# databendlabs/databend

Measured on AMD Instinct MI355X. Metric: rows/s TPC-H Q1 hash-agg, higher is better.
Workload: dtype i64/i128 decimal

## Files before the change

databend_amd/csrc/k_decimal.hip:

```cpp
#include "dev_common.h"
#include "dev_decimal.h"
#include "dev_load.h"
#include "runtime.h"

using namespace dbhip;

namespace {

struct DecParams : DecOp {
  const void* a;
  const void* b;
  void* out;
  const uint8_t* a_validity;
  const uint8_t* b_validity;
  int64_t a_voff, b_voff;
  int64_t n;
  uint32_t* err_words;
  unsigned long long* err_count;
  int a_type, b_type, out_type;
  int a_scalar, b_scalar;
};

__device__ __forceinline__ i128 load_operand(const void* p, int type, bool scalar, int64_t i) {
  int64_t j = scalar ? 0 : i;
  switch (type) {
    case DBHIP_T_DEC128: return ((const i128*)p)[j];
    case DBHIP_T_DEC256: return ((const i128*)p)[2 * j];
    case DBHIP_T_DEC64: case DBHIP_T_I64: return (i128)((const int64_t*)p)[j];
    case DBHIP_T_I8: return (i128)((const int8_t*)p)[j];
    case DBHIP_T_I16: return (i128)((const int16_t*)p)[j];
    case DBHIP_T_I32: return (i128)((const int32_t*)p)[j];
    case DBHIP_T_U8: return (i128)((const uint8_t*)p)[j];
    case DBHIP_T_U16: return (i128)((const uint16_t*)p)[j];
    case DBHIP_T_U32: return (i128)((const uint32_t*)p)[j];
    default: return (i128)((const uint64_t*)p)[j];
  }
}

__device__ __forceinline__ void dec_raise(const DecParams& p, int64_t row) {
  if (p.a_validity && !bit_get(p.a_validity, p.a_voff + (p.a_scalar ? 0 : row))) return;
  if (p.b_validity && !bit_get(p.b_validity, p.b_voff + (p.b_scalar ? 0 : row))) return;
  if (p.err_words) atomicAnd(&p.err_words[row >> 5], ~(1u << (row & 31)));
  if (p.err_count) atomicAdd(p.err_count, 1ULL);
}

template <int N>
__device__ __forceinline__ void load_operand_n(const void* p, int type, bool scalar, const int64_t (&i)[N], i128 (&out)[N]) {
  int64_t j[N];
#pragma unroll
  for (int u = 0; u < N; ++u) j[u] = scalar ? 0 : i[u];
  switch (type) {
    case DBHIP_T_DEC128:
#pragma unroll
      for (int u = 0; u < N; ++u) out[u] = ((const i128*)p)[j[u]];
      break;
    case DBHIP_T_DEC256:
#pragma unroll
      for (int u = 0; u < N; ++u) out[u] = ((const i128*)p)[2 * j[u]];
      break;
    case DBHIP_T_DEC64: case DBHIP_T_I64:
#pragma unroll
      for (int u = 0; u < N; ++u) out[u] = (i128)((const int64_t*)p)[j[u]];
      break;
    case DBHIP_T_I8:
#pragma unroll
      for (int u = 0; u < N; ++u) out[u] = (i128)((const int8_t*)p)[j[u]];
      break;
    case DBHIP_T_I16:
#pragma unroll
      for (int u = 0; u < N; ++u) out[u] = (i128)((const int16_t*)p)[j[u]];
      break;
    case DBHIP_T_I32:
#pragma unroll
      for (int u = 0; u < N; ++u) out[u] = (i128)((const int32_t*)p)[j[u]];
      break;
    case DBHIP_T_U8:
#pragma unroll
      for (int u = 0; u < N; ++u) out[u] = (i128)((const uint8_t*)p)[j[u]];
      break;
    case DBHIP_T_U16:
#pragma unroll
      for (int u = 0; u < N; ++u) out[u] = (i128)((const uint16_t*)p)[j[u]];
      break;
    case DBHIP_T_U32:
#pragma unroll
      for (int u = 0; u < N; ++u) out[u] = (i128)((const uint32_t*)p)[j[u]];
      break;
    default:
#pragma unroll
      for (int u = 0; u < N; ++u) out[u] = (i128)((const uint64_t*)p)[j[u]];
      break;
  }
}

__global__ __launch_bounds__(256) void decimal_kernel(DecParams p) {
  const bool t128 = p.t_is_128;
  const bool a_dec = p.a_type == DBHIP_T_DEC64 || p.a_type == DBHIP_T_DEC128 || p.a_type == DBHIP_T_DEC256;
  const bool b_dec = p.b_type == DBHIP_T_DEC64 || p.b_type == DBHIP_T_DEC128 || p.b_type == DBHIP_T_DEC256;
  constexpr int U = 4;
  const int64_t T = (int64_t)gridDim.x * blockDim.x;
  const int64_t t = (int64_t)blockIdx.x * blockDim.x + threadIdx.x;
  for (int64_t base = 0; base < p.n; base += U * T) {
    int64_t row[U];
    bool in[U];
#pragma unroll
    for (int u = 0; u < U; ++u) {
      row[u] = base + u * T + t;
      in[u] = row[u] < p.n;
      if (!in[u]) row[u] = p.n - 1;
    }
    i128 av[U], bv[U];
    load_operand_n<U>(p.a, p.a_type, p.a_scalar, row, av);
    load_operand_n<U>(p.b, p.b_type, p.b_scalar, row, bv);
#pragma unroll
    for (int u = 0; u < U; ++u) {
      if (!in[u]) continue;
      const int64_t i = row[u];
      i128 r;
      if (!dec_row(p, av[u], bv[u], a_dec, b_dec, t128, &r)) {
        dec_raise(p, i);
        r = 1;
      }
      if (p.out_type == DBHIP_T_DEC128) ((i128*)p.out)[i] = r;
      else ((int64_t*)p.out)[i] = (int64_t)r;
    }
  }
}

struct DSize {
  int p, s;
};

bool decimal_props(int type, int prec, int scale, DSize* out) {
  switch (type) {
    case DBHIP_T_DEC64: case DBHIP_T_DEC128: case DBHIP_T_DEC256: *out = {prec, scale}; return prec >= 1 && prec <= 76 && scale <= prec;
    case DBHIP_T_I8: case DBHIP_T_U8: *out = {3, 0}; return true;
    case DBHIP_T_I16: case DBHIP_T_U16: *out = {5, 0}; return true;
    case DBHIP_T_I32: case DBHIP_T_U32: *out = {10, 0}; return true;
    case DBHIP_T_I64: *out = {19, 0}; return true;
    case DBHIP_T_U64: *out = {20, 0}; return true;
  }
  return false;
}

inline int imin(int a, int b) { return a < b ? a : b; }
inline int imax(int a, int b) { return a > b ? a : b; }

bool result_size(int op, DSize a, DSize b, DSize* left, DSize* right, DSize* ret) {
  int precision, scale;
  int la = a.p - a.s, lb = b.p - b.s;
  switch (op) {
    case DBHIP_OP_MULTIPLY:
      scale = imin(a.s + b.s, imax(imax(a.s, b.s), 12));
      precision = la + lb + scale;
      break;
    case DBHIP_OP_DIVIDE:
      scale = imax(a.s, imin(a.s + 6, 12));
      precision = la + b.s + scale;
      break;
    case DBHIP_OP_PLUS:
    case DBHIP_OP_MINUS:
      scale = imax(a.s, b.s);
      precision = imax(la, lb) + scale + 1;
      break;
    default:
      return false;
  }
  precision = imin(precision, (a.p <= 38 && b.p <= 38) ? 38 : 76);
  if (precision < 1 || scale > precision) return false;
  *ret = {precision, scale};
  switch (op) {
    case DBHIP_OP_MULTIPLY:
      *left = {precision, a.s};
      *right = {precision, b.s};
      break;
    case DBHIP_OP_DIVIDE: {
      int pp = imax(precision, imax(a.p, b.p));
      *left = {pp, a.s};
      *right = {pp, b.s};
    } break;
    default:
      *left = *ret;
      *right = *ret;
  }
  return left->s <= left->p && right->s <= right->p;
}

}

namespace dbhip {
int32_t decimal256_arith(int32_t op, const dbhip_col* lhs, const dbhip_col* rhs, int64_t n, int32_t out_type, uint8_t out_precision,
                         uint8_t out_scale, void* out, uint8_t* err_bitmap, uint64_t* err_count_dev, void* stream);
}

extern "C" {

int32_t dbhip_decimal_result_size(int32_t op, uint8_t lp, uint8_t ls, uint8_t rp, uint8_t rs,
                                  uint8_t* out_precision_host, uint8_t* out_scale_host) {
  DSize l, r, ret;
  if (!result_size(op, {lp, ls}, {rp, rs}, &l, &r, &ret)) {
    set_error("dbhip_decimal_result_size: no decimal result for op %d on (%d,%d),(%d,%d)", op, lp, ls, rp, rs);
    return DBHIP_ERR_INVALID;
  }
  if (out_precision_host) *out_precision_host = (uint8_t)ret.p;
  if (out_scale_host) *out_scale_host = (uint8_t)ret.s;
  return DBHIP_OK;
}

int32_t dbhip_decimal_arith(int32_t op, const dbhip_col* lhs, const dbhip_col* rhs, int64_t n,
                            int32_t out_type, uint8_t out_precision, uint8_t out_scale, void* out,
                            uint8_t* err_bitmap, uint64_t* err_count_dev, void* stream) {
  DBHIP_REQUIRE(lhs && rhs && (out || n == 0), "dbhip_decimal_arith: NULL argument");
  if (out_precision > 38)
    return decimal256_arith(op, lhs, rhs, n, out_type, out_precision, out_scale, out, err_bitmap, err_count_dev, stream);
  DecParams p;
  int want_type, rp, rs;
  int32_t rc = dbhip_decimal_decode_internal(op, lhs->type, lhs->precision, lhs->scale, rhs->type, rhs->precision, rhs->scale, &p,
                                             &want_type, &rp, &rs);
  if (rc) return rc;
  if (rp != out_precision || rs != out_scale || want_type != out_type) {
    set_error("dbhip_decimal_arith: result is type %d Decimal(%d,%d); caller passed type %d Decimal(%d,%d)",
              want_type, rp, rs, out_type, out_precision, out_scale);
    return DBHIP_ERR_INVALID;
  }
  hipStream_t s = resolve_stream(stream);
  if (err_bitmap) DBHIP_CHECK(hipMemsetAsync(err_bitmap, 0xFF, (size_t)ceil_div(n, 32) * 4, s));
  if (n == 0) return DBHIP_OK;
  p.a = lhs->data; p.b = rhs->data; p.out = out;
  p.a_validity = lhs->validity; p.b_validity = rhs->validity;
  p.a_voff = lhs->validity_offset; p.b_voff = rhs->validity_offset;
  p.n = n;
  p.err_words = (uint32_t*)err_bitmap;
  p.err_count = (unsigned long long*)err_count_dev;
  p.a_type = lhs->type; p.b_type = rhs->type; p.out_type = out_type;
  p.a_scalar = lhs->is_scalar; p.b_scalar = rhs->is_scalar;
  hipLaunchKernelGGL(decimal_kernel, dim3(grid_for(ceil_div(n, 4), 256, 1024)), dim3(256), 0, s, p);
  DBHIP_LAUNCH_CHECK();
  return DBHIP_OK;
}

}

int32_t dbhip_decimal_decode_internal(int op, int a_type, int a_prec, int a_scale, int b_type, int b_prec, int b_scale,
                                      DecOp* out, int* out_type, int* out_precision, int* out_scale) {
  DSize a, b, left, right, ret;
  if (!decimal_props(a_type, a_prec, a_scale, &a) || !decimal_props(b_type, b_prec, b_scale, &b)) {
    set_error("decimal arithmetic: operand types (%d,%d) have no decimal properties", a_type, b_type);
    return DBHIP_ERR_INVALID;
  }
  const bool a_dec = a_type == DBHIP_T_DEC64 || a_type == DBHIP_T_DEC128 || a_type == DBHIP_T_DEC256;
  const bool b_dec = b_type == DBHIP_T_DEC64 || b_type == DBHIP_T_DEC128 || b_type == DBHIP_T_DEC256;
  DBHIP_REQUIRE(a_dec || b_dec, "decimal arithmetic: at least one side must be decimal");
  if (!result_size(op, a, b, &left, &right, &ret)) {
    set_error("decimal arithmetic: unsupported op %d", op);
    return DBHIP_ERR_INVALID;
  }
  if (ret.p > 38) {
    set_error("decimal arithmetic: Decimal(%d,%d) results (T = i256) are evaluated by dbhip_decimal_arith, not inside fused programs", ret.p, ret.s);
    return DBHIP_ERR_UNSUPPORTED;
  }
  DecOp& p = *out;
  p.op = op;
  p.a_from_scale = a.s; p.a_to_scale = left.s; p.a_to_precision = left.p;
  p.a_check = a_dec ? (a.s != left.s) : 1;
  p.b_from_scale = b.s; p.b_to_scale = right.s; p.b_to_precision = right.p;
  p.b_check = b_dec ? (b.s != right.s) : 1;
  p.t_is_128 = ret.p > 18;
  p.ret_precision = ret.p; p.ret_scale = ret.s;
  p.overflow = ret.p == (p.t_is_128 ? 38 : 18);
  p.scale_mul = op == DBHIP_OP_MULTIPLY ? a.s + b.s - ret.s
                                        : (op == DBHIP_OP_DIVIDE ? b.s + ret.s - a.s : 0);
  if (p.scale_mul < 0 || p.scale_mul > 38) {
    set_error("decimal arithmetic: scale shift %d outside the supported range", p.scale_mul);
    return DBHIP_ERR_UNSUPPORTED;
  }
  {
    const bool pass_a = a_dec ? !p.a_check : p.a_to_scale == 0, pass_b = b_dec ? !p.b_check : p.b_to_scale == 0;
    p.trivial = pass_a && pass_b && (((op == DBHIP_OP_PLUS || op == DBHIP_OP_MINUS) && !p.overflow) || (op == DBHIP_OP_MULTIPLY && p.scale_mul == 0));
  }
  *out_type = ret.p <= 18 ? DBHIP_T_DEC64 : DBHIP_T_DEC128;
  *out_precision = ret.p;
  *out_scale = ret.s;
  return DBHIP_OK;
}
```

Before: 90.72 billion.

## Add specialized fast decimal add/sub/mul kernel with templated operand kinds

Adds a templated fast-path decimal kernel for plus, minus and multiply without division. It specializes on operand kind (scalar, 64-bit, 128-bit, narrow int) and result width, precomputes rescale factors on the host, and uses vectorized 16-byte loads and stores in a grid-stride chunked loop. The aim is to remove the runtime type dispatch and generic 128-bit arithmetic of the general kernel. In exchange it adds many template instantiations, alignment requirements, and a duplicated overflow and rescale logic path that must match the generic semantics.

After: 90.71 billion (median of 2 runs). Within noise of the previous version (-0.0%).

```diff
diff --git a/databend_amd/csrc/dev_decimal_fast.h b/databend_amd/csrc/dev_decimal_fast.h
--- /dev/null
+++ b/databend_amd/csrc/dev_decimal_fast.h
@@ -0,0 +1,123 @@
+#pragma once
+#include "dev_decimal.h"
+
+struct DecFastSide {
+  i128 mul;
+  i128 max;
+  int rescale;
+  int uns;
+};
+
+struct DecFastOp {
+  DecFastSide a, b;
+  i128 ret_max;
+  int overflow;
+};
+
+__host__ inline bool dec_fast_decode(const DecOp& p, bool a_dec, bool b_dec, bool a_u64, bool b_u64, DecFastOp* f) {
+  if (dec_op_needs_division(p)) return false;
+  const bool ra = a_dec ? p.a_check != 0 : p.a_to_scale != 0, rb = b_dec ? p.b_check != 0 : p.b_to_scale != 0;
+  if (p.op == DBHIP_OP_MULTIPLY && (ra || rb)) return false;
+  const int ka = a_dec ? p.a_to_scale - p.a_from_scale : p.a_to_scale, kb = b_dec ? p.b_to_scale - p.b_from_scale : p.b_to_scale;
+  if ((ra && (ka < 0 || ka > 38)) || (rb && (kb < 0 || kb > 38))) return false;
+  if (!p.t_is_128 && ((ra && ka > 18) || (rb && kb > 18))) return false;
+  f->a = {ra ? pow10_i128(ka) : (i128)1, max_for_precision(p.a_to_precision), ra, a_u64};
+  f->b = {rb ? pow10_i128(kb) : (i128)1, max_for_precision(p.b_to_precision), rb, b_u64};
+  f->ret_max = max_for_precision(p.ret_precision);
+  f->overflow = p.overflow;
+  return true;
+}
+
+__host__ __device__ __forceinline__ bool decf_convert(const DecFastSide& s, int64_t x, int64_t* out) {
+  if (!s.rescale) {
+    *out = x;
+    return true;
+  }
+  const i128 r = (i128)x * (i128)(int64_t)s.mul;
+  *out = (int64_t)r;
+  return r <= s.max && r >= -s.max;
+}
+
+__host__ __device__ __forceinline__ bool decf_mag_mul64(uint64_t ax, u128 f, u128 max, u128* out) {
+  const u128 lo = (u128)ax * (uint64_t)f;
+  const u128 hi = (u128)ax * (uint64_t)(f >> 64) + (uint64_t)(lo >> 64);
+  *out = (hi << 64) | (uint64_t)lo;
+  return (uint64_t)(hi >> 64) == 0 && *out <= max;
+}
+__host__ __device__ __forceinline__ bool decf_mag_mul128(u128 ax, u128 f, u128 max, u128* out) {
+  const u256 pr = u256_mul_128(ax, f);
+  *out = pr.lo;
+  return pr.hi == 0 && pr.lo <= max;
+}
+
+__host__ __device__ __forceinline__ bool decf_convert(const DecFastSide& s, int64_t x, i128* out) {
+  const bool neg = !s.uns && x < 0;
+  if (!s.rescale) {
+    *out = (i128)(((u128)(neg ? ~0ULL : 0ULL) << 64) | (uint64_t)x);
+    return true;
+  }
+  u128 m;
+  const bool ok = decf_mag_mul64(neg ? (uint64_t)0 - (uint64_t)x : (uint64_t)x, (u128)s.mul, (u128)s.max, &m);
+  *out = neg ? (i128)((u128)0 - m) : (i128)m;
+  return ok;
+}
+__host__ __device__ __forceinline__ bool decf_convert(const DecFastSide& s, i128 x, i128* out) {
+  if (!s.rescale) {
+    *out = x;
+    return true;
+  }
+  const bool neg = x < 0;
+  u128 m;
+  const bool ok = decf_mag_mul128(neg ? (u128)0 - (u128)x : (u128)x, (u128)s.mul, (u128)s.max, &m);
+  *out = neg ? (i128)((u128)0 - m) : (i128)m;
+  return ok;
+}
+
+__host__ __device__ __forceinline__ i128 decf_mul128(int64_t a, bool a_uns, int64_t b, bool b_uns) {
+  const u128 p = (u128)(uint64_t)a * (uint64_t)b;
+  uint64_t hi = (uint64_t)(p >> 64);
+  if (!a_uns && a < 0) hi -= (uint64_t)b;
+  if (!b_uns && b < 0) hi -= (uint64_t)a;
+  return (i128)(((u128)hi << 64) | (uint64_t)p);
+}
+__host__ __device__ __forceinline__ i128 decf_mul128(i128 a, bool, int64_t b, bool b_uns) {
+  const uint64_t al = (uint64_t)(u128)a, ah = (uint64_t)((u128)a >> 64);
+  const u128 p = (u128)al * (uint64_t)b;
+  uint64_t hi = (uint64_t)(p >> 64) + ah * (uint64_t)b;
+  if (!b_uns && b < 0) hi -= al;
+  return (i128)(((u128)hi << 64) | (uint64_t)p);
+}
+__host__ __device__ __forceinline__ i128 decf_mul128(int64_t a, bool a_uns, i128 b, bool b_uns) { return decf_mul128(b, b_uns, a, a_uns); }
+__host__ __device__ __forceinline__ i128 decf_mul128(i128 a, bool, i128 b, bool) { return (i128)((u128)a * (u128)b); }
+
+template <typename T>
+struct decf_unsigned;
+template <>
+struct decf_unsigned<int64_t> {
+  typedef uint64_t type;
+};
+template <>
+struct decf_unsigned<i128> {
+  typedef u128 type;
+};
+
+template <typename T, int OP, bool A_PRE, bool B_PRE, typename AT, typename BT>
+__host__ __device__ __forceinline__ bool dec_row_fast(const DecFastOp& p, AT av, bool a_ok, BT bv, bool b_ok, T* out) {
+  typedef typename decf_unsigned<T>::type UT;
+  if constexpr (OP == DBHIP_OP_MULTIPLY) {
+    if constexpr (sizeof(T) == 8) *out = (T)((UT)av * (UT)bv);
+    else *out = decf_mul128(av, p.a.uns != 0, bv, p.b.uns != 0);
+    return (A_PRE ? a_ok : true) & (B_PRE ? b_ok : true);
+  } else {
+    T a, b;
+    bool ok = true;
+    if constexpr (A_PRE) { a = (T)av; ok = a_ok; }
+    else ok = decf_convert(p.a, av, &a);
+    if constexpr (B_PRE) { b = (T)bv; ok = b_ok & ok; }
+    else ok = decf_convert(p.b, bv, &b) & ok;
+    const T t = OP == DBHIP_OP_PLUS ? (T)((UT)a + (UT)b) : (T)((UT)a - (UT)b);
+    if (p.overflow) ok = ok & (t <= (T)p.ret_max) & (t >= -(T)p.ret_max);
+    *out = t;
+    return ok;
+  }
+}
diff --git a/databend_amd/csrc/k_decimal.hip b/databend_amd/csrc/k_decimal.hip
--- a/databend_amd/csrc/k_decimal.hip
+++ b/databend_amd/csrc/k_decimal.hip
@@ -1,5 +1,6 @@
 #include "dev_common.h"
 #include "dev_decimal.h"
+#include "dev_decimal_fast.h"
 #include "dev_load.h"
 #include "runtime.h"
 
@@ -125,6 +126,193 @@
       else ((int64_t*)p.out)[i] = (int64_t)r;
     }
   }
+}
+
+enum { DK_SCALAR = 0, DK_C64 = 1, DK_C128 = 2, DK_NARROW = 3 };
+constexpr int DF_BLOCK = 256;
+constexpr int DF_PAIRS = 4;
+constexpr int DF_CHUNK_ROWS = DF_BLOCK * 2 * DF_PAIRS;
+constexpr int DF_GRID_CAP = 512;
+
+struct DecFastParams : DecParams {
+  DecFastOp f;
+};
+
+typedef int64_t df_i64x2 __attribute__((ext_vector_type(2)));
+typedef uint32_t df_u32x4 __attribute__((ext_vector_type(4)));
+
+template <int K, typename T> struct df_operand { typedef int64_t type; };
+template <typename T> struct df_operand<DK_C128, T> { typedef i128 type; };
+template <typename T> struct df_operand<DK_SCALAR, T> { typedef T type; };
+
+__device__ __forceinline__ int64_t df_load_narrow(const void* p, int type, int64_t i) {
+  switch (type) {
+    case DBHIP_T_I8: return ((const int8_t*)p)[i];
+    case DBHIP_T_I16: return ((const int16_t*)p)[i];
+    case DBHIP_T_I32: return ((const int32_t*)p)[i];
+    case DBHIP_T_U8: return ((const uint8_t*)p)[i];
+    case DBHIP_T_U16: return ((const uint16_t*)p)[i];
+    default: return ((const uint32_t*)p)[i];
+  }
+}
+
+__device__ __forceinline__ i128 df_i128(df_u32x4 w) {
+  return (i128)(((u128)(((uint64_t)w.w << 32) | w.z) << 64) | (((uint64_t)w.y << 32) | w.x));
+}
+__device__ __forceinline__ df_u32x4 df_words(i128 v) {
+  const uint64_t lo = (uint64_t)(u128)v, hi = (uint64_t)((u128)v >> 64);
+  df_u32x4 w = {(uint32_t)lo, (uint32_t)(lo >> 32), (uint32_t)hi, (uint32_t)(hi >> 32)};
+  return w;
+}
+
+template <int K, typename V>
+__device__ __forceinline__ void df_load_chunk(const void* base, int type, int64_t chunk, uint32_t tid, V (&v)[2 * DF_PAIRS]) {
+  if constexpr (K == DK_C64) {
+    const char* cb = (const char*)base + chunk * (int64_t)(DF_CHUNK_ROWS * 8);
+#pragma unroll
+    for (int u = 0; u < DF_PAIRS; ++u) {
+      const df_i64x2 x = *(const df_i64x2*)(cb + (uint32_t)((u * DF_BLOCK + tid) * 16u));
+      v[2 * u] = x.x;
+      v[2 * u + 1] = x.y;
+    }
+  } else if constexpr (K == DK_C128) {
+    const char* cb = (const char*)base + chunk * (int64_t)(DF_CHUNK_ROWS * 16);
+#pragma unroll
+    for (int k = 0; k < 2 * DF_PAIRS; ++k)
+            v[k] = df_i128(*(const df_u32x4*)(cb + (uint32_t)((((k >> 1) * DF_BLOCK + tid) * 2u + (k & 1)) * 16u)));
+  } else if constexpr (K == DK_NARROW) {
+    const int64_t r0 = chunk * DF_CHUNK_ROWS;
+#pragma unroll
+    for (int k = 0; k < 2 * DF_PAIRS; ++k) v[k] = df_load_narrow(base, type, r0 + ((k >> 1) * DF_BLOCK + tid) * 2 + (k & 1));
+  }
+}
+
+template <int K, typename V>
+__device__ __forceinline__ V df_load_row(const void* base, int type, int64_t row) {
+  if constexpr (K == DK_C64) return ((const int64_t*)base)[row];
+  else if constexpr (K == DK_C128) return ((const i128*)base)[row];
+  else return df_load_narrow(base, type, row);
+}
+
+template <typename T, int OP, int AK, int BK>
+__global__ __launch_bounds__(DF_BLOCK) void decimal_fast_kernel(DecFastParams p) {
+  typedef typename df_operand<AK, T>::type AT;
+  typedef typename df_operand<BK, T>::type BT;
+  constexpr bool A_PRE = AK == DK_SCALAR, B_PRE = BK == DK_SCALAR;
+  const uint32_t tid = threadIdx.x;
+  T sa = 0, sb = 0;
+  bool a_ok = true, b_ok = true;
+  if constexpr (A_PRE) {
+    const bool a_dec = p.a_type == DBHIP_T_DEC64 || p.a_type == DBHIP_T_DEC128;
+    i128 c = 0;
+    a_ok = convert_operand(load_operand(p.a, p.a_type, true, 0), a_dec, p.a_from_scale, p.a_to_scale, p.a_to_precision, p.a_check, sizeof(T) == 16, &c);
+    sa = (T)c;
+  }
+  if constexpr (B_PRE) {
+    const bool b_dec = p.b_type == DBHIP_T_DEC64 || p.b_type == DBHIP_T_DEC128;
+    i128 c = 0;
+    b_ok = convert_operand(load_operand(p.b, p.b_type, true, 0), b_dec, p.b_from_scale, p.b_to_scale, p.b_to_precision, p.b_check, sizeof(T) == 16, &c);
+    sb = (T)c;
+  }
+  const int64_t n_chunks = (p.n + DF_CHUNK_ROWS - 1) / DF_CHUNK_ROWS;
+  for (int64_t chunk = blockIdx.x; chunk < n_chunks; chunk += gridDim.x) {
+    const int64_t r0 = chunk * DF_CHUNK_ROWS;
+    if (r0 + DF_CHUNK_ROWS <= p.n) {
+      AT av[2 * DF_PAIRS];
+      BT bv[2 * DF_PAIRS];
+      if constexpr (A_PRE) {
+#pragma unroll
+        for (int k = 0; k < 2 * DF_PAIRS; ++k) av[k] = sa;
+      } else {
+        df_load_chunk<AK>(p.a, p.a_type, chunk, tid, av);
+      }
+      if constexpr (B_PRE) {
+#pragma unroll
+        for (int k = 0; k < 2 * DF_PAIRS; ++k) bv[k] = sb;
+      } else {
+        df_load_chunk<BK>(p.b, p.b_type, chunk, tid, bv);
+      }
+      T r[2 * DF_PAIRS];
+      uint32_t raised = 0;
+#pragma unroll
+      for (int k = 0; k < 2 * DF_PAIRS; ++k) {
+        const bool ok = dec_row_fast<T, OP, A_PRE, B_PRE>(p.f, av[k], a_ok, bv[k], b_ok, &r[k]);
+        r[k] = ok ? r[k] : (T)1;
+        raised |= ok ? 0u : 1u << k;
+      }
+      if (raised) {
+#pragma unroll 1
+        for (int k = 0; k < 2 * DF_PAIRS; ++k)
+          if ((raised >> k) & 1) dec_raise(p, r0 + ((k >> 1) * DF_BLOCK + tid) * 2 + (k & 1));
+      }
+      char* ob = (char*)p.out + r0 * (int64_t)sizeof(T);
+      if constexpr (sizeof(T) == 8) {
+#pragma unroll
+        for (int u = 0; u < DF_PAIRS; ++u) {
+          df_i64x2 x = {(int64_t)r[2 * u], (int64_t)r[2 * u + 1]};
+          *(df_i64x2*)(ob + (uint32_t)((u * DF_BLOCK + tid) * 16u)) = x;
+        }
+      } else {
+#pragma unroll
+        for (int k = 0; k < 2 * DF_PAIRS; ++k)
+          *(df_u32x4*)(ob + (uint32_t)((((k >> 1) * DF_BLOCK + tid) * 2u + (k & 1)) * 16u)) = df_words(r[k]);
+      }
+    } else {
+      for (int64_t row = r0 + tid; row < p.n; row += DF_BLOCK) {
+        AT a;
+        BT b;
+        if constexpr (A_PRE) a = sa;
+        else a = df_load_row<AK, AT>(p.a, p.a_type, row);
+        if constexpr (B_PRE) b = sb;
+        else b = df_load_row<BK, BT>(p.b, p.b_type, row);
+        T r;
+        if (!dec_row_fast<T, OP, A_PRE, B_PRE>(p.f, a, a_ok, b, b_ok, &r)) {
+          dec_raise(p, row);
+          r = 1;
+        }
+        ((T*)p.out)[row] = r;
+      }
+    }
+  }
+}
+
+typedef void (*DfKernel)(DecFastParams);
+
+template <typename T, int OP>
+DfKernel df_pick_kinds(int ak, int bk) {
+#define DF_CASE(A, B) \
+  if (ak == A && bk == B) return decimal_fast_kernel<T, OP, A, B>;
+  DF_CASE(DK_SCALAR, DK_C64) DF_CASE(DK_C64, DK_SCALAR) DF_CASE(DK_C64, DK_C64) DF_CASE(DK_NARROW, DK_C64) DF_CASE(DK_C64, DK_NARROW)
+  if constexpr (sizeof(T) == 16) {
+    DF_CASE(DK_SCALAR, DK_C128) DF_CASE(DK_C128, DK_SCALAR) DF_CASE(DK_C64, DK_C128) DF_CASE(DK_C128, DK_C64) DF_CASE(DK_C128, DK_C128)
+    DF_CASE(DK_NARROW, DK_C128) DF_CASE(DK_C128, DK_NARROW)
+  }
+#undef DF_CASE
+  return nullptr;
+}
+
+template <typename T>
+DfKernel df_pick(int op, int ak, int bk) {
+  switch (op) {
+    case DBHIP_OP_PLUS: return df_pick_kinds<T, DBHIP_OP_PLUS>(ak, bk);
+    case DBHIP_OP_MINUS: return df_pick_kinds<T, DBHIP_OP_MINUS>(ak, bk);
+    case DBHIP_OP_MULTIPLY: return df_pick_kinds<T, DBHIP_OP_MULTIPLY>(ak, bk);
+  }
+  return nullptr;
+}
+
+int df_kind(const dbhip_col* c, bool t128) {
+  int k;
+  switch (c->type) {
+    case DBHIP_T_DEC64: k = DK_C64; break;
+    case DBHIP_T_I64: case DBHIP_T_U64: if (!t128) return -1; k = DK_C64; break;
+    case DBHIP_T_DEC128: if (!t128) return -1; k = DK_C128; break;
+    case DBHIP_T_I8: case DBHIP_T_I16: case DBHIP_T_I32: case DBHIP_T_U8: case DBHIP_T_U16: case DBHIP_T_U32: k = DK_NARROW; break;
+    default: return -1;
+  }
+  if (c->is_scalar) return DK_SCALAR;
+  if (k != DK_NARROW && ((uintptr_t)c->data & 15)) return -1;
+  return k;
 }
 
 struct DSize {
@@ -234,6 +422,20 @@
   p.err_count = (unsigned long long*)err_count_dev;
   p.a_type = lhs->type; p.b_type = rhs->type; p.out_type = out_type;
   p.a_scalar = lhs->is_scalar; p.b_scalar = rhs->is_scalar;
+  if (!dec_op_needs_division(p) && ((uintptr_t)out & 15) == 0) {
+    const bool t128 = p.t_is_128;
+    const int ak = df_kind(lhs, t128), bk = df_kind(rhs, t128);
+    DecFastParams fp;
+    static_cast<DecParams&>(fp) = p;
+    DfKernel k = ak < 0 || bk < 0 ? nullptr : (t128 ? df_pick<i128>(op, ak, bk) : df_pick<int64_t>(op, ak, bk));
+    if (k && dec_fast_decode(p, lhs->type == DBHIP_T_DEC64 || lhs->type == DBHIP_T_DEC128, rhs->type == DBHIP_T_DEC64 || rhs->type == DBHIP_T_DEC128,
+                             lhs->type == DBHIP_T_U64, rhs->type == DBHIP_T_U64, &fp.f)) {
+      void* args[] = {&fp};
+      DBHIP_CHECK(hipLaunchKernel((const void*)k, dim3(grid_for(ceil_div(n, 2 * DF_PAIRS), DF_BLOCK, DF_GRID_CAP)), dim3(DF_BLOCK), args, 0, s));
+      DBHIP_LAUNCH_CHECK();
+      return DBHIP_OK;
+    }
+  }
   hipLaunchKernelGGL(decimal_kernel, dim3(grid_for(ceil_div(n, 4), 256, 1024)), dim3(256), 0, s, p);
   DBHIP_LAUNCH_CHECK();
   return DBHIP_OK;
```

## Add templated streaming decimal kernel with nontemporal loads and lean fast path

Applied to the files above, without the earlier changes.

Adds a wave-per-chunk streaming kernel, templated on operand kind (scalar, 8-byte, 16-byte) and result width, for non-division decimal ops on aligned columns. It uses nontemporal loads and stores with a coalesced lane+64k layout, and a lean variant that drops overflow and rescale checks when type analysis shows they cannot trigger. The aim is to cut per-row type dispatch and cache pollution in the memory-bound arithmetic ahead of the aggregation. It adds many template instantiations, and correctness relies on the lean predicate being right.

Measured after the change: 94.11 billion before, 94.03 billion after. About the same (-0.1%).

```diff
diff --git a/databend_amd/csrc/k_decimal.hip b/databend_amd/csrc/k_decimal.hip
--- a/databend_amd/csrc/k_decimal.hip
+++ b/databend_amd/csrc/k_decimal.hip
@@ -124,6 +124,128 @@
       if (p.out_type == DBHIP_T_DEC128) ((i128*)p.out)[i] = r;
       else ((int64_t*)p.out)[i] = (int64_t)r;
     }
+  }
+}
+
+enum { DK_SCALAR = 0, DK_8 = 1, DK_16 = 2 };
+constexpr int kStreamRows = 7;
+constexpr int kStreamBlock = 256;
+constexpr int kStreamGridCap = 1024;
+
+template <int K>
+__device__ __forceinline__ i128 stream_load(const void* p, int64_t base, uint32_t off) {
+  if constexpr (K == DK_16) return __builtin_nontemporal_load((const i128*)p + base + off);
+  else return (i128)__builtin_nontemporal_load((const int64_t*)p + base + off);
+}
+
+template <int KA, int KB, bool T128, bool FULL>
+__device__ __forceinline__ void stream_chunk(const DecParams& p, const DecOp& q, int64_t base, uint32_t lane, i128 as, i128 bs, bool a_dec, bool b_dec) {
+  constexpr int R = kStreamRows;
+  uint32_t off[R];
+#pragma unroll
+  for (int k = 0; k < R; ++k) {
+    off[k] = lane + 64u * k;
+    if (!FULL && base + off[k] >= p.n) off[k] = (uint32_t)(p.n - 1 - base);
+  }
+  i128 av[R], bv[R];
+#pragma unroll
+  for (int k = 0; k < R; ++k) {
+    if constexpr (KA == DK_SCALAR) av[k] = as;
+    else av[k] = stream_load<KA>(p.a, base, off[k]);
+  }
+#pragma unroll
+  for (int k = 0; k < R; ++k) {
+    if constexpr (KB == DK_SCALAR) bv[k] = bs;
+    else bv[k] = stream_load<KB>(p.b, base, off[k]);
+  }
+#pragma unroll
+  for (int k = 0; k < R; ++k) {
+    if (!FULL && base + lane + 64u * k >= p.n) continue;
+    i128 r;
+    if (!dec_row_nodiv(q, av[k], bv[k], a_dec, b_dec, T128, &r)) {
+      dec_raise(p, base + off[k]);
+      r = 1;
+    }
+    if constexpr (T128) __builtin_nontemporal_store(r, (i128*)p.out + base + off[k]);
+    else __builtin_nontemporal_store((int64_t)r, (int64_t*)p.out + base + off[k]);
+  }
+}
+
+template <int KA, int KB, bool T128, bool LEAN>
+__global__ __launch_bounds__(kStreamBlock) void decimal_stream_kernel(DecParams p) {
+  constexpr int64_t C = 64 * kStreamRows;
+  const bool a_dec = p.a_type == DBHIP_T_DEC64 || p.a_type == DBHIP_T_DEC128 || p.a_type == DBHIP_T_DEC256;
+  const bool b_dec = p.b_type == DBHIP_T_DEC64 || p.b_type == DBHIP_T_DEC128 || p.b_type == DBHIP_T_DEC256;
+  DecOp q = p;
+  if constexpr (LEAN) {
+    q.overflow = 0;
+    if constexpr (KA != DK_SCALAR) { q.a_check = 0; q.a_to_scale = 0; }
+    if constexpr (KB != DK_SCALAR) { q.b_check = 0; q.b_to_scale = 0; }
+  }
+  const uint32_t lane = threadIdx.x & 63;
+  const int wave_in_block = __builtin_amdgcn_readfirstlane((int)(threadIdx.x >> 6));
+  const int64_t wave = (int64_t)blockIdx.x * (kStreamBlock / 64) + wave_in_block;
+  const int64_t waves = (int64_t)gridDim.x * (kStreamBlock / 64);
+  const int64_t chunks = (p.n + C - 1) / C;
+  i128 as = 0, bs = 0;
+  if constexpr (KA == DK_SCALAR) as = load_operand(p.a, p.a_type, true, 0);
+  if constexpr (KB == DK_SCALAR) bs = load_operand(p.b, p.b_type, true, 0);
+  for (int64_t c = wave; c < chunks; c += waves) {
+    const int64_t base = c * C;
+    if (LEAN && base + C <= p.n) stream_chunk<KA, KB, T128, true>(p, q, base, lane, as, bs, a_dec, b_dec);
+    else stream_chunk<KA, KB, T128, false>(p, q, base, lane, as, bs, a_dec, b_dec);
+  }
+}
+
+int stream_kind(const dbhip_col* c) {
+  if (c->is_scalar) return DK_SCALAR;
+  if ((uintptr_t)c->data & 15) return -1;
+  switch (c->type) {
+    case DBHIP_T_DEC64: case DBHIP_T_I64: return DK_8;
+    case DBHIP_T_DEC128: return DK_16;
+  }
+  return -1;
+}
+
+bool stream_is_lean(const DecParams& p, bool a_dec, bool b_dec) {
+  const bool pass_a = p.a_scalar || (a_dec ? !p.a_check : p.a_to_scale == 0);
+  const bool pass_b = p.b_scalar || (b_dec ? !p.b_check : p.b_to_scale == 0);
+  return pass_a && pass_b && (p.op == DBHIP_OP_MULTIPLY || !p.overflow);
+}
+
+template <int KA, int KB>
+bool launch_stream(const DecParams& p, bool lean, int grid, hipStream_t s) {
+  const dim3 g(grid), b(kStreamBlock);
+  if (p.t_is_128) {
+    if (lean) {
+      if constexpr (KA == DK_8 && KB == DK_8) return false;
+      else hipLaunchKernelGGL((decimal_stream_kernel<KA, KB, true, true>), g, b, 0, s, p);
+    } else {
+      hipLaunchKernelGGL((decimal_stream_kernel<KA, KB, true, false>), g, b, 0, s, p);
+    }
+  } else {
+    if (lean) hipLaunchKernelGGL((decimal_stream_kernel<KA, KB, false, true>), g, b, 0, s, p);
+    else hipLaunchKernelGGL((decimal_stream_kernel<KA, KB, false, false>), g, b, 0, s, p);
+  }
+  return true;
+}
+
+bool launch_stream(int ka, int kb, const DecParams& p, hipStream_t s) {
+  const bool a_dec = p.a_type == DBHIP_T_DEC64 || p.a_type == DBHIP_T_DEC128 || p.a_type == DBHIP_T_DEC256;
+  const bool b_dec = p.b_type == DBHIP_T_DEC64 || p.b_type == DBHIP_T_DEC128 || p.b_type == DBHIP_T_DEC256;
+  const bool lean = stream_is_lean(p, a_dec, b_dec);
+  const int64_t chunks = ceil_div(p.n, 64 * kStreamRows);
+  const int grid = (int)std::min<int64_t>(ceil_div(chunks, kStreamBlock / 64), kStreamGridCap);
+  switch (ka * 3 + kb) {
+    case 0: return launch_stream<DK_SCALAR, DK_SCALAR>(p, lean, grid, s);
+    case 1: return launch_stream<DK_SCALAR, DK_8>(p, lean, grid, s);
+    case 2: return launch_stream<DK_SCALAR, DK_16>(p, lean, grid, s);
+    case 3: return launch_stream<DK_8, DK_SCALAR>(p, lean, grid, s);
+    case 4: return launch_stream<DK_8, DK_8>(p, lean, grid, s);
+    case 5: return launch_stream<DK_8, DK_16>(p, lean, grid, s);
+    case 6: return launch_stream<DK_16, DK_SCALAR>(p, lean, grid, s);
+    case 7: return launch_stream<DK_16, DK_8>(p, lean, grid, s);
+    default: return launch_stream<DK_16, DK_16>(p, lean, grid, s);
   }
 }
 
@@ -234,7 +356,12 @@
   p.err_count = (unsigned long long*)err_count_dev;
   p.a_type = lhs->type; p.b_type = rhs->type; p.out_type = out_type;
   p.a_scalar = lhs->is_scalar; p.b_scalar = rhs->is_scalar;
-  hipLaunchKernelGGL(decimal_kernel, dim3(grid_for(ceil_div(n, 4), 256, 1024)), dim3(256), 0, s, p);
+  const int ka = stream_kind(lhs), kb = stream_kind(rhs);
+  bool streamed = false;
+  if (!dec_op_needs_division(p) && ka >= 0 && kb >= 0 && ((uintptr_t)out & 15) == 0)
+    streamed = launch_stream(ka, kb, p, s);
+  if (!streamed)
+    hipLaunchKernelGGL(decimal_kernel, dim3(grid_for(ceil_div(n, 4), 256, 1024)), dim3(256), 0, s, p);
   DBHIP_LAUNCH_CHECK();
   return DBHIP_OK;
 }
```
